# microsoft/Spartan2

Measured on AMD Instinct MI355X. Metric: sha256_spartan prove(): R1CS constraints/sec (prove wall-clock in ms_per_step), higher is better.
Workload: dtype u256 modular integer (8 x u32 Montgomery limbs; T256 scalar/base fields)

## Files before the change

spartan2_amd/csrc/capi_core.hip:

```cpp
#include <atomic>
#include <chrono>
#include <cstdlib>
#include <cstdio>
#include <cstring>

#include "core.hpp"
#include "walk_pool.hpp"
#include "kernels_poly.hpp"
#include "sumcheck_round.hpp"

namespace sp {
static thread_local std::string g_err;
static thread_local sp_wait_hook g_wait_hook = nullptr;
static thread_local void* g_wait_user = nullptr;
void set_error(const std::string& m) { g_err = m; }
static std::atomic<int> g_live_contexts{0};
int live_contexts() { return g_live_contexts.load(std::memory_order_relaxed); }
void relax() {
  if (g_wait_hook) g_wait_hook(g_wait_user);
  else __builtin_ia32_pause();
}
void slow_note(const char* site, long spins) {
  static const bool on = getenv("SPARTAN_SLOWPATH_LOG") != nullptr;
  if (on) fprintf(stderr, "[slow path] %s after %ld polls\n", site, spins);
// ... 501 lines not shown
  if (cap_bytes) *cap_bytes = t->cap * sizeof(fe_t);
  return SP_OK;
}
void sp_table_free(sp_table* t) {
  if (!t) return;
  if (t->d && !t->view) hipFree(t->d);
  delete t;
}

}

static int launch_bind(sp_ctx* c, sp_table** tabs, int nt, const fe_t& r) {
  if (nt > spk::BIND_MAX_TABLES) return fail(SP_ERR_INTERNAL, "launch_bind: too many tables");
  spk::BindArgs a;
  size_t max_eff = 0;
  uint64_t bytes = 0;
  for (int i = 0; i < nt; ++i) {
    sp_table* t = tabs[i];
    if (t->len < 2) return fail(SP_ERR_INVALID_INPUT_LENGTH, "bind_poly_var_top: table must have at least two elements");
    a.z[i] = t->d;
    a.n[i] = t->len / 2;
    a.lo[i] = sp::eff_lo(t);
    a.hi[i] = sp::eff_hi(t);
    size_t eff = sp::eff_pairs(t);
    if (eff > max_eff) max_eff = eff;
    bytes += 48ull * t->len;
  }
  a.r = r;
  a.one_minus_r = fe_sub<S>(fe_one<S>(), r);
  if (max_eff > 0) {
    size_t blocks = (max_eff + 255) / 256;
    if (blocks > 8192) blocks = 8192;
    dim3 grid((unsigned)blocks, (unsigned)nt);
    c->timed("bind", bytes, [&] { hipLaunchKernelGGL(spk::k_bind_top, grid, dim3(256), 0, c->stream, a); });
  }
  for (int i = 0; i < nt; ++i) sp::after_bind(tabs[i]);
  return SP_OK;
}

static unsigned next_seq(sp_ctx* c) { return ++c->result_seq; }
static void reduce_partials_launch(sp_ctx* c, size_t nblocks, int nacc) {
  if (nblocks <= (size_t)spk::HOST_SUM_MAX_BLOCKS) {
    c->pending_slots = (unsigned)nblocks;
    return;
  }
  size_t b2 = (nblocks + 63) / 64;
  if (b2 > (size_t)spk::HOST_SUM_MAX_BLOCKS) b2 = spk::HOST_SUM_MAX_BLOCKS;
  c->pending_slots = (unsigned)b2;
  hipLaunchKernelGGL(spk::k_sum_partials, dim3((unsigned)b2), dim3(64), 0, c->stream, c->d_scratch, nblocks, nacc, c->d_pinned, c->result_seq);
}
static bool fold_stage2_enabled() {
  static const bool on = [] {
    const char* e = getenv("SPARTAN_FOLD_STAGE2");
    return e && e[0] == '1';
  }();
  return on;
}
static spk::LazyOut lazy_out(sp_ctx* c, spk::lazy9_t* lp, size_t nparts, int gl, const fe_t* eq_out, unsigned seq) {
  spk::LazyOut lo(lp);
  const size_t ngroups = nparts >> gl;
  size_t b2 = (ngroups + 63) / 64;
  if (b2 < 1) b2 = 1;
  if (b2 > (size_t)spk::HOST_SUM_MAX_BLOCKS) b2 = spk::HOST_SUM_MAX_BLOCKS;
  lo.eq_out = eq_out;
  lo.mapped = c->d_pinned;
  lo.seq = seq;
  lo.nslots = (unsigned)b2;
  lo.gl = gl;
  static const unsigned fold_slots = [] {
    const char* e = getenv("SPARTAN_FOLD_SLOTS");
    const int v = e ? atoi(e) : spk::HOST_SUM_MAX_BLOCKS;
    return (unsigned)(v < 1 ? 1 : (v > spk::HOST_SUM_MAX_BLOCKS ? spk::HOST_SUM_MAX_BLOCKS : v));
  }();
  size_t fs = fold_slots;
  while (fs > 1 && (fs > ngroups || ngroups % fs)) fs >>= 1;
  const bool even = ngroups > 0 && ((size_t)ngroups << gl) == nparts && ngroups % fs == 0 && (gl == 0 || nparts % 2 == 0);
  if (fold_stage2_enabled() && even && c->d_fold_tickets) {
    lo.tickets = c->d_fold_tickets;
    lo.nslots = (unsigned)fs;
    lo.per_slot = (unsigned)(nparts / fs);
  }
  return lo;
}
static void sum_lazy_launch(sp_ctx* c, const spk::LazyOut& lo, size_t nparts) {
  const int gl = lo.gl;
  const unsigned seq = lo.seq;
  const fe_t* eq_out = lo.eq_out;
  c->pending_slots = lo.nslots;
  if (lo.tickets) return;
  const uint32_t* P = reinterpret_cast<const uint32_t*>(lo.P);
  const dim3 g(lo.nslots), b(64);
  const bool vec_ok = nparts % 8 == 0;
  if (vec_ok && gl == 0) hipLaunchKernelGGL((spk::k_sum_partials_lazy<0>), g, b, 0, c->stream, P, nparts, gl, eq_out, c->d_pinned, seq);
  else if (vec_ok && gl == 1) hipLaunchKernelGGL((spk::k_sum_partials_lazy<1>), g, b, 0, c->stream, P, nparts, gl, eq_out, c->d_pinned, seq);
  else if (vec_ok && gl == 2) hipLaunchKernelGGL((spk::k_sum_partials_lazy<2>), g, b, 0, c->stream, P, nparts, gl, eq_out, c->d_pinned, seq);
  else if (vec_ok && gl == 3) hipLaunchKernelGGL((spk::k_sum_partials_lazy<3>), g, b, 0, c->stream, P, nparts, gl, eq_out, c->d_pinned, seq);
  else hipLaunchKernelGGL((spk::k_sum_partials_lazy<-1>), g, b, 0, c->stream, P, nparts, gl, eq_out, c->d_pinned, seq);
}
static int wait_slot(sp_ctx* c, const fe_t* slot, unsigned want, int nvals, fe_t* v, bool resident, long* spins) {
  volatile const unsigned* fl = reinterpret_cast<volatile const unsigned*>(slot + 3);
  while (*fl != want) {
    if (++*spins > 400000) {
      sp::slow_note("wait_slot", *spins);
      if (resident) {
        const auto t0 = std::chrono::steady_clock::now();
        while (*fl != want) {
          if (std::chrono::steady_clock::now() - t0 > std::chrono::seconds(12)) return fail(SP_ERR_INTERNAL, "sum-check tail kernel did not deliver a round result");
          sp::relax();
        }
        break;
      }
      SP_HIP(sp::stream_sync(c->stream));
      if (*fl != want) return fail(SP_ERR_INTERNAL, "evaluation kernel did not deliver its block sums");
    }
    sp::relax();
  }
  for (long tries = 0;; ++tries) {
    std::atomic_thread_fence(std::memory_order_acquire);
    spk::slot_chk chk = {want, want * spk::SLOT_CHK_K};
    for (int k = 0; k < nvals; ++k) {
      for (int i = 0; i < 8; ++i) v[k].v[i] = reinterpret_cast<volatile const uint32_t*>(slot + k)[i];
      spk::slot_chk_add(chk, v[k], k);
    }
    if (fl[0] == want && fl[1] == chk.a && fl[2] == chk.b && fl[3] == want) return SP_OK;
    if (tries > 4000000) return fail(SP_ERR_INTERNAL, "evaluation kernel delivered an inconsistent result slot");
    sp::relax();
  }
}
int sp::wait_result_slot(sp_ctx* c, const fe_t* slot, unsigned want, int nvals, fe_t* v, long* spins) { return wait_slot(c, slot, want, nvals, v, false, spins); }
static int wait_wide(sp_ctx* c, unsigned want, int nvals, fe_t* v) {
  long spins = 0;
  for (int s0 = 0; s0 < nvals; s0 += 3) {
    int rc = wait_slot(c, c->h_pinned + spk::SLOT_BASE_ELEM + 4 * (s0 / 3), want, nvals - s0 < 3 ? nvals - s0 : 3, v + s0, true, &spins);
    if (rc) return rc;
  }
  return SP_OK;
}
static unsigned host_parts(size_t items, size_t min_per_part) {
  const size_t w = (size_t)sp::WalkPool::get().walkers() + 1;
  size_t p = items / min_per_part;
  if (p > w) p = w;
  if (p > (size_t)sp::WalkPool::MAX_PARTS) p = sp::WalkPool::MAX_PARTS;
  return p ? (unsigned)p : 1u;
}
static int wait_hand_over(sp_ctx* c, unsigned want, int nvals, fe_t* v) {
  long spins = 0;
  const fe_t* area = c->h_pinned + spk::HAND_BASE_ELEM;
  int rc = wait_slot(c, area, want, nvals < 3 ? nvals : 3, v, true, &spins);
  if (rc) return rc;
  for (int s0 = 3; s0 < nvals; s0 += 3) {
    const char* line = reinterpret_cast<const char*>(area + 4 * (s0 / 3));
    __builtin_prefetch(line);
    __builtin_prefetch(line + 64);
  }
  const int nslots = (nvals + 2) / 3;
  if (nslots > 48 && sp::WalkPool::get().walkers() > 0) {
    struct Check {
      sp_ctx* c;
      const fe_t* area;
      unsigned want;
      int nvals, nslots;
      fe_t* v;
      std::atomic<int> rc{SP_OK};
    } ck{c, area, want, nvals, nslots, v};
    auto part = [](void* arg, unsigned p, unsigned np) {
      Check& k = *static_cast<Check*>(arg);
      const int lo = 1 + (int)((long)(k.nslots - 1) * p / np), hi = 1 + (int)((long)(k.nslots - 1) * (p + 1) / np);
      long sp_ = 0;
      for (int sl = lo; sl < hi; ++sl) {
        const int s0 = 3 * sl;
        const int r = wait_slot(k.c, k.area + 4 * sl, k.want, k.nvals - s0 < 3 ? k.nvals - s0 : 3, k.v + s0, true, &sp_);
        if (r) k.rc.store(r, std::memory_order_relaxed);
      }
// ... 782 lines not shown
      }
      return 1;
    }
    if (round + 1 >= rounds) {
      if (ahead) return 0;
      sp_table* tabs[2] = {A, B};
      have_sums = false;
      int rc2 = launch_bind(c, tabs, 2, rv);
      return rc2 ? rc2 : 1;
    }
    const bool gated = ahead && !launch_ahead_ok(c, A->len);
    if (gated && !gate_ok(c)) return 0;
    if (!stopped && tail_enabled() && A->len <= TAIL_MAX_LEN && table_dense(A) && table_dense(B) && lease.take(tail_blocks(A->len / 2))) {
      spk::TailArgs ta;
      ta.A = A->d;
      ta.B = B->d;
      ta.C = nullptr;
      ta.len = A->len;
      ta.r0 = rv;
      ta.eq_pl = ta.eq_pr = nullptr;
      ta.ell = ta.first_half = ta.rnd0 = 0;
      ta.mail = c->d_mail;
      ta.mirror = c->d_mail_mirror;
      ta.r0_from_mail = ahead ? 1 : 0;
      ta.mapped = c->d_pinned;
      ta.seq0 = next_seq(c);
      ta.hand_n = tail_hand_n(false);
      tail_nb0 = tail_blocks(A->len / 2);
      hipLaunchKernelGGL((spk::k_sumcheck_tail<false>), dim3(tail_nb0), dim3(spk::TAIL_THREADS), 0, c->stream, ta);
      if (!c->tail_ev) (void)hipEventCreateWithFlags(&c->tail_ev, hipEventDisableTiming);
      if (c->tail_ev && hipEventRecord(c->tail_ev, c->stream) == hipSuccess) c->tail_ev_pending = true;
      in_tail = true;
      have_sums = true;
      sp::after_bind(A);
      sp::after_bind(B);
      c->pending_slots = tail_blocks(A->len);
      return 1;
    }
    const bool dense = table_dense(A) && table_dense(B);
    const bool sparse_stream = !dense && A->len / 4 >= STREAM_MIN_Q && sp::eff_lo(A) == A->len / 2 && sp::eff_lo(B) == B->len / 2 && sp::eff_hi(A) <= A->len / 4 && sp::eff_hi(B) <= B->len / 4;
    if (gated && !dense && !sparse_stream) return 0;
    const spk::MailRef mref = gated ? gate_launch(c, answers) : mail_ref(c, ahead, answers);
    if (dense) {
      const size_t q = A->len / 4;
      size_t blocks = (q + chunk - 1) / chunk;
      if (q >= STREAM_MIN_Q) {
        const unsigned seq = next_seq(c);
        const spk::LazyOut lp = lazy_out(c, reinterpret_cast<spk::lazy9_t*>(c->d_scratch), q / 256, 2, nullptr, seq);
        c->timed("bind_stream_quad", 48ull * A->len * 2, [&] {
          hipLaunchKernelGGL(spk::k_bind_eval_quad_stream, dim3((unsigned)(q / 256)), dim3(256), 0, c->stream, A->d, B->d, q, rv, lp, mref);
        });
        sum_lazy_launch(c, lp, q / 256);
      } else {
        c->timed("bind", 48ull * A->len * 2, [&] {
          hipLaunchKernelGGL(spk::k_bind_eval_quad, dim3((unsigned)blocks), dim3(256), 0, c->stream, A->d, B->d, q, rv, c->d_scratch, c->d_pinned, next_seq(c), mref);
        });
        reduce_partials_launch(c, blocks, 2);
      }
      sp::after_bind(A);
      sp::after_bind(B);
      have_sums = true;
      return 1;
    }
    if (sparse_stream) {
      const size_t q = A->len / 4;
      const unsigned seq = next_seq(c);
      const spk::LazyOut lp = lazy_out(c, reinterpret_cast<spk::lazy9_t*>(c->d_scratch), q / 256, 2, nullptr, seq);
      c->timed("bind_stream_quad_sparse", 64ull * (A->len / 2) * 2, [&] {
        hipLaunchKernelGGL(spk::k_bind_eval_quad_stream_sparse, dim3((unsigned)(q / 256)), dim3(256), 0, c->stream, A->d, B->d, q, rv, sp::eff_hi(A), sp::eff_hi(B), lp,
                           mref);
      });
      sum_lazy_launch(c, lp, q / 256);
      sp::after_bind(A);
      sp::after_bind(B);
      have_sums = true;
      return 1;
    }
    if (ahead) return 0;
    sp_table* tabs[2] = {A, B};
    have_sums = false;
    int rc2 = launch_bind(c, tabs, 2, rv);
    return rc2 ? rc2 : 1;
  };
  for (size_t round = 0; round < rounds; ++round) {
    const size_t half = A->len / 2, len_now = A->len;
    const double tr0 = round_trace() ? now_us() : 0;
    fe_t sums[2] = {fe_zero(), fe_zero()};
    bool waiting = have_sums;
    if (!have_sums && !host_mode) {
      size_t len = sp::eff_pairs(A);
      if (sp::eff_pairs(B) < len) len = sp::eff_pairs(B);
      if (half < len) len = half;
      if (len >= STREAM_MIN_Q && len % 1024 == 0) {
        const unsigned seq = next_seq(c);
        const size_t hi_max = sp::eff_hi(A) > sp::eff_hi(B) ? sp::eff_hi(A) : sp::eff_hi(B);
        const bool lowhi = hi_max <= len / 2;
        const size_t blocks = len / (256 * (size_t)4);
        const spk::LazyOut lp = lazy_out(c, reinterpret_cast<spk::lazy9_t*>(c->d_scratch), blocks, 2, nullptr, seq);
        c->timed("eval_quad", 64ull * len + 32ull * ((sp::eff_hi(A) < len ? sp::eff_hi(A) : len) + (sp::eff_hi(B) < len ? sp::eff_hi(B) : len)), [&] {
          if (lowhi)
            hipLaunchKernelGGL((spk::k_eval_quad_stream_lowhi<4>), dim3((unsigned)blocks), dim3(256), 0, c->stream, A->d, B->d, half, sp::eff_hi(A), sp::eff_hi(B), lp);
          else
            hipLaunchKernelGGL((spk::k_eval_quad_stream<4>), dim3((unsigned)blocks), dim3(256), 0, c->stream, A->d, B->d, half, sp::eff_hi(A), sp::eff_hi(B), lp);
        });
        sum_lazy_launch(c, lp, blocks);
        waiting = true;
      } else if (len > 0) {
        size_t blocks = (len + chunk - 1) / chunk;
        c->timed("eval_quad", 64ull * len + 32ull * ((sp::eff_hi(A) < len ? sp::eff_hi(A) : len) + (sp::eff_hi(B) < len ? sp::eff_hi(B) : len)),
                 [&] { hipLaunchKernelGGL(spk::k_eval_quad, dim3((unsigned)blocks), dim3(256), 0, c->stream, A->d, B->d, half, len, sp::eff_hi(A), sp::eff_hi(B), c->d_scratch, c->d_pinned, next_seq(c)); });
        reduce_partials_launch(c, blocks, 2);
        waiting = true;
      }
    }
    const unsigned wait_seq = c->result_seq, wait_slots = c->pending_slots;
    const bool wait_resident = in_tail;
    if (wait_resident && !host_mode && spk::tail_hand_over(len_now, tail_hand_n(false))) {
      hA.resize(2 * len_now);
      if ((rc = wait_hand_over(c, wait_seq, (int)(2 * len_now), hA.data()))) return rc;
      hB = hA.data() + len_now;
      host_mode = true;
      hand_seq = wait_seq;
    }
    if (host_mode) {
      host_quad_eval(hA.data(), hB, half, sums);
      waiting = false;
    }
    if (!host_mode && wait_resident && spk::tail_double(false, len_now, tail_hand_n(false))) {
      fe_t S8[8];
      if ((rc = wait_wide(c, wait_seq, spk::TAIL_DOUBLE_SUMS_QUAD, S8))) return rc;
      if (reduce) {
        int hrc = reduce(reduce_user, reinterpret_cast<uint64_t*>(S8), 8);
        if (hrc) return fail(hrc, "prove_quad: the reduce hook failed");
      }
      fe_t rr[2];
      for (int half2 = 0; half2 < 2; ++half2) {
        fe_t e0, tinf;
        if (half2 == 0) {
          e0 = fe_add<S>(S8[0], S8[1]);
          tinf = fe_add<S>(S8[2], S8[3]);
        } else {
          const fe_t r = rr[0];
          e0 = fe_add<S>(S8[0], fe_mul<S>(r, fe_add<S>(fe_sub<S>(fe_sub<S>(S8[4], S8[0]), S8[2]), fe_mul<S>(r, S8[2]))));
          tinf = fe_add<S>(S8[5], fe_mul<S>(r, fe_add<S>(fe_sub<S>(fe_sub<S>(S8[7], S8[5]), S8[6]), fe_mul<S>(r, S8[6]))));
        }
        UniPoly poly;
        poly.n = 3;
        poly.c[0] = e0;
        poly.c[1] = fe_sub<S>(fe_sub<S>(claim, fe_dbl<S>(e0)), tinf);
        poly.c[2] = tinf;
        absorb_poly(tr->t, poly);
        if (!tr->t.squeeze<S>(lbl_c, 1, &rr[half2])) return fail(SP_ERR_INTERNAL_TRANSCRIPT, "transcript round counter overflow");
        tail_post_challenge(c, rr[half2], wait_seq + half2);
        store_fe(out_r + 4 * (round + half2), rr[half2]);
        store_fe(out_cpolys + 8 * (round + half2), poly.c[0]);
        store_fe(out_cpolys + 8 * (round + half2) + 4, poly.c[2]);
        claim = poly_eval(poly, rr[half2]);
      }
      for (int k = 0; k < 2; ++k) {
        sp::after_bind(A);
        sp::after_bind(B);
        next_seq(c);
      }
      have_sums = round + 2 < rounds;
      c->pending_slots = have_sums ? 1u : 0u;
      last_answered = wait_seq + 1;
      guard.armed = round + 2 < rounds;
      if (observe)
        for (int k = 0; k < 2; ++k) {
          uint64_t rw[4];
          store_fe(rw, rr[k]);
          observe(observe_user, round + k, rw);
        }
      if (round_trace()) fprintf(stderr, "quad rounds %2zu+%2zu len %8zu tail 2 wait+host %7.1f us\n", round, round + 1, len_now, now_us() - tr0);
      ++round;
      continue;
    }
    int issued = 0;
    if (!host_mode && waiting && (in_tail || (c->mail_dev && !reduce))) {
      issued = issue(round, nullptr, wait_seq);
      if (issued < 0) return issued;
      guard.armed = issued != 0;
    }
    if (waiting) {
      const unsigned cur_seq = c->result_seq, cur_slots = c->pending_slots;
      c->result_seq = wait_seq;
      c->pending_slots = wait_slots;
      rc = reduce_partials_wait(c, 2, sums, wait_resident || issued != 0);
      if (issued) {
        c->result_seq = cur_seq;
        c->pending_slots = cur_slots;
      }
      if (rc) return rc;
    }
    if (reduce) {
      int hrc = reduce(reduce_user, reinterpret_cast<uint64_t*>(sums), 2);
      if (hrc) return fail(hrc, "prove_quad: the reduce hook failed");
    }
    const double tr1 = round_trace() ? now_us() : 0;
    fe_t e0 = sums[0], tinf = sums[1];
    UniPoly poly;
    poly.n = 3;
    poly.c[0] = e0;
    poly.c[1] = fe_sub<S>(fe_sub<S>(claim, fe_dbl<S>(e0)), tinf);
    poly.c[2] = tinf;
    absorb_poly(tr->t, poly);
    fe_t r_i;
    if (!tr->t.squeeze<S>(lbl_c, 1, &r_i)) return fail(SP_ERR_INTERNAL_TRANSCRIPT, "transcript round counter overflow");
    last_answered = wait_seq;
    if (host_mode) {
      host_bind_tables(hA.data(), (size_t)(hB - hA.data()), 2, len_now, r_i);
      sp::after_bind(A);
      sp::after_bind(B);
      have_sums = false;
    } else if (issued) {
      tail_post_challenge(c, r_i, wait_seq);
    } else {
      issued = issue(round, &r_i, wait_seq);
      if (issued < 0) return issued;
      if (wait_resident) tail_post_challenge(c, r_i, wait_seq);
    }
    store_fe(out_r + 4 * round, r_i);
    store_fe(out_cpolys + 8 * round, poly.c[0]);
    store_fe(out_cpolys + 8 * round + 4, poly.c[2]);
    claim = poly_eval(poly, r_i);
    guard.armed = in_tail && (host_mode || round + 1 < rounds);
    if (observe) {
      uint64_t rw[4];
      store_fe(rw, r_i);
      observe(observe_user, round, rw);
    }
    if (round_trace()) fprintf(stderr, "quad round %2zu len %8zu tail %d wait %7.1f us host %6.1f us\n", round, len_now, (int)wait_resident, tr1 - tr0, now_us() - tr1);
  }
  if (stopped) {
    store_fe(claim_io, claim);
    return tail_check(c);
  }
  if (host_mode) {
    store_fe(out_final, hA[0]);
    store_fe(out_final + 4, hB[0]);
    tail_post_challenge(c, hA[0], hand_seq);
    tail_post_challenge(c, hB[0], hand_seq + 1);
    c->result_seq = hand_seq + 1;
    guard.armed = false;
  } else if (in_tail) {
    fe_t fin[3];
    long spins = 0;
    if ((rc = wait_slot(c, c->h_pinned + spk::TAIL_FINAL_ELEM, last_answered, 2, fin, true, &spins))) return rc;
    store_fe(out_final, fin[0]);
    store_fe(out_final + 4, fin[1]);
  } else {
    rc = sp_table_read(c, A, 0, 1, out_final);
    if (rc) return rc;
    rc = sp_table_read(c, B, 0, 1, out_final + 4);
    if (rc) return rc;
  }
// ... 1077 lines not shown
```

spartan2_amd/csrc/kernels_poly.hpp:

```cpp
#pragma once
#include "device_utils.hpp"
#include "kernels_shared.hpp"

namespace spk {

constexpr int RESULT_FLAG_ELEM = 7;
__device__ __forceinline__ void publish_result(fe_t* result, unsigned seq) {
  __threadfence_system();
  __hip_atomic_store(reinterpret_cast<unsigned*>(result + RESULT_FLAG_ELEM), seq, __ATOMIC_RELEASE, __HIP_MEMORY_SCOPE_SYSTEM);
}

template <int NACC>
__device__ __forceinline__ void emit_partials_wide(const fe_t (&acc)[NACC], fe_t* __restrict__ mapped, unsigned seq);
template <int NACC>
__device__ __forceinline__ void emit_partials(const fe_t (&acc)[NACC], fe_t* __restrict__ partials, fe_t* __restrict__ mapped, unsigned seq) {
  if (gridDim.x <= HOST_SUM_MAX_BLOCKS) {
    fe_t* slot = mapped + SLOT_BASE_ELEM + 4 * blockIdx.x;
    slot_chk chk = {0u, 0u};
#pragma unroll
    for (int k = 0; k < NACC; ++k) {
      slot_store_elem(slot + k, acc[k]);
      slot_chk_add(chk, acc[k], k);
    }
    slot_store_tag(slot, seq, chk);
// ... 488 lines not shown
  bool nz = false;
#pragma unroll
  for (int k = 0; k < PPT; ++k) nz |= !fe_is_zero(p0[k]);
  lazy9_t l0 = lazy_from(fe_zero()), l1 = lazy_from(fe_zero());
#pragma unroll
  for (int k = 0; k < PPT; ++k) l1 = lazy_add(l1, lazy_from(fe_mul<S>(w[k], p1[k])));
  l1 = lazy_wave_sum(l1);
  if (__any(nz)) {
#pragma unroll
    for (int k = 0; k < PPT; ++k) l0 = lazy_add(l0, lazy_from(fe_mul<S>(w[k], p0[k])));
    l0 = lazy_wave_sum(l0);
  }
  stream_block_partials(l0, l1, partials);
}
__global__ void __launch_bounds__(256) k_bind_eval_quad_stream(fe_t* __restrict__ A, fe_t* __restrict__ B, size_t q, fe_t r_arg, LazyOut partials,
                                                               MailRef mref) {
  const size_t id = (size_t)blockIdx.x * blockDim.x + threadIdx.x;
  const fe_t la0 = A[id], la1 = A[id + q], la2 = A[id + 2 * q], la3 = A[id + 3 * q];
  const fe_t lb0 = B[id], lb1 = B[id + q], lb2 = B[id + 2 * q], lb3 = B[id + 3 * q];
  const fe_t r = challenge_or(mref, r_arg);
  const fe_t a0 = bind1(la0, la2, r), a1 = bind1(la1, la3, r);
  const fe_t b0 = bind1(lb0, lb2, r), b1 = bind1(lb1, lb3, r);
  A[id] = a0;
  A[id + q] = a1;
  B[id] = b0;
  B[id + q] = b1;
  stream_block_partials(lazy_wave_sum(lazy_from(fe_mul<S>(a0, b0))), lazy_wave_sum(lazy_from(fe_mul<S>(fe_sub<S>(a1, a0), fe_sub<S>(b1, b0)))), partials);
}
__global__ void __launch_bounds__(256) k_bind_eval_quad_stream_sparse(fe_t* __restrict__ A, fe_t* __restrict__ B, size_t q, fe_t r_arg, size_t hiA, size_t hiB,
                                                                      LazyOut partials, MailRef mref) {
  const size_t id = (size_t)blockIdx.x * blockDim.x + threadIdx.x;
  const fe_t la0 = A[id], la1 = A[id + q], lb0 = B[id], lb1 = B[id + q];
  const fe_t r = challenge_or(mref, r_arg);
  const fe_t one_minus_r = fe_sub<S>(fe_one<S>(), r);
  const fe_t a0 = id < hiA ? bind1(la0, A[id + 2 * q], r) : fe_mul<S>(la0, one_minus_r);
  const fe_t b0 = id < hiB ? bind1(lb0, B[id + 2 * q], r) : fe_mul<S>(lb0, one_minus_r);
  const fe_t a1 = fe_mul<S>(la1, one_minus_r), b1 = fe_mul<S>(lb1, one_minus_r);
  A[id] = a0;
  A[id + q] = a1;
  B[id] = b0;
  B[id + q] = b1;
  stream_block_partials(lazy_wave_sum(lazy_from(fe_mul<S>(a0, b0))), lazy_wave_sum(lazy_from(fe_mul<S>(fe_sub<S>(a1, a0), fe_sub<S>(b1, b0)))), partials);
}
template <int PPT>
__global__ void __launch_bounds__(256) k_eval_quad_stream(const fe_t* __restrict__ A, const fe_t* __restrict__ B, size_t half, size_t hiA, size_t hiB,
                                                          LazyOut partials) {
  const size_t stride = (size_t)gridDim.x * blockDim.x;
  size_t id = (size_t)blockIdx.x * blockDim.x + threadIdx.x;
  lazy9_t l0 = lazy_from(fe_zero()), l1 = lazy_from(fe_zero());
#pragma unroll
  for (int k = 0; k < PPT; ++k, id += stride) {
    const fe_t a0 = A[id], b0 = B[id];
    const fe_t a1 = id < hiA ? A[id + half] : fe_zero(), b1 = id < hiB ? B[id + half] : fe_zero();
    l0 = lazy_add(l0, lazy_from(fe_mul<S>(a0, b0)));
    l1 = lazy_add(l1, lazy_from(fe_mul<S>(fe_sub<S>(a1, a0), fe_sub<S>(b1, b0))));
  }
  stream_block_partials(lazy_wave_sum(l0), lazy_wave_sum(l1), partials);
}
template <int PPT>
__global__ void __launch_bounds__(256) k_eval_quad_stream_lowhi(const fe_t* __restrict__ A, const fe_t* __restrict__ B, size_t half, size_t hiA, size_t hiB,
                                                                LazyOut partials) {
  const size_t stride = (size_t)gridDim.x * blockDim.x;
  const size_t id0 = (size_t)blockIdx.x * blockDim.x + threadIdx.x;
  fe_t a0[PPT], b0[PPT];
#pragma unroll
  for (int k = 0; k < PPT; ++k) {
    a0[k] = A[id0 + k * stride];
    b0[k] = B[id0 + k * stride];
  }
  lazy9_t l0 = lazy_from(fe_zero()), l1 = lazy_from(fe_zero());
#pragma unroll
  for (int k = 0; k < PPT; ++k) {
    const size_t id = id0 + k * stride;
    const fe_t p = fe_mul<S>(a0[k], b0[k]);
    l0 = lazy_add(l0, lazy_from(p));
    if (id < hiA || id < hiB) {
      const fe_t a1 = id < hiA ? A[id + half] : fe_zero(), b1 = id < hiB ? B[id + half] : fe_zero();
      l1 = lazy_add(l1, lazy_from(fe_sub<S>(fe_mul<S>(fe_sub<S>(a1, a0[k]), fe_sub<S>(b1, b0[k])), p)));
    }
  }
  l1 = lazy_add(l1, l0);
  stream_block_partials(lazy_wave_sum(l0), lazy_wave_sum(l1), partials);
}
template <int GL>
__global__ void __launch_bounds__(64) k_sum_partials_lazy(const uint32_t* __restrict__ P, size_t nparts, int gl_rt, const fe_t* __restrict__ eq_out,
                                                          fe_t* __restrict__ mapped, unsigned seq) {
  const int gl = GL >= 0 ? GL : gl_rt;
  const size_t ngroups = nparts >> gl, per = (size_t)1 << gl;
  fe_t acc[2] = {fe_zero(), fe_zero()};
  for (size_t g = (size_t)blockIdx.x * 64 + threadIdx.x; g < ngroups; g += (size_t)gridDim.x * 64) {
    unsigned long long col[2][9];
#pragma unroll
    for (int w = 0; w < 9; ++w)
#pragma unroll
      for (int a = 0; a < 2; ++a) {
        const uint32_t* src = P + (size_t)(2 * w + a) * nparts + g * per;
        if constexpr (GL == 0) {
          col[a][w] = src[0];
        } else if constexpr (GL == 1) {
          const uint2 v = *reinterpret_cast<const uint2*>(src);
          col[a][w] = (unsigned long long)v.x + v.y;
        } else if constexpr (GL == 2) {
          const uint4 v = *reinterpret_cast<const uint4*>(src);
          col[a][w] = ((unsigned long long)v.x + v.y) + ((unsigned long long)v.z + v.w);
        } else if constexpr (GL == 3) {
          const uint4 v = *reinterpret_cast<const uint4*>(src), u = *reinterpret_cast<const uint4*>(src + 4);
          col[a][w] = (((unsigned long long)v.x + v.y) + ((unsigned long long)v.z + v.w)) + (((unsigned long long)u.x + u.y) + ((unsigned long long)u.z + u.w));
        } else {
          unsigned long long t = 0;
          for (size_t k = 0; k < per; ++k) t += src[k];
          col[a][w] = t;
        }
      }
    fe_t f[2];
#pragma unroll
    for (int a = 0; a < 2; ++a) {
      lazy9_t l;
      unsigned long long carry = 0;
#pragma unroll
      for (int w = 0; w < 9; ++w) {
        const unsigned long long t = col[a][w] + carry;
        l.v[w] = (uint32_t)t;
        carry = t >> 32;
      }
      f[a] = lazy_reduce(l);
    }
    if (eq_out) {
      const fe_t eo = eq_out[g];
      f[0] = fe_mul<S>(f[0], eo);
      f[1] = fe_mul<S>(f[1], eo);
    }
    acc[0] = fe_add<S>(acc[0], f[0]);
    acc[1] = fe_add<S>(acc[1], f[1]);
  }
  acc[0] = wave_sum(acc[0]);
  acc[1] = wave_sum(acc[1]);
  if (threadIdx.x == 0) emit_partials<2>(acc, nullptr, mapped, seq);
}

__global__ void __launch_bounds__(256) k_eval_quad(const fe_t* __restrict__ A, const fe_t* __restrict__ B, size_t half, size_t len, size_t hiA, size_t hiB,
                                                   fe_t* __restrict__ partials, fe_t* __restrict__ single_out, unsigned seq) {
  __shared__ fe_t smem[2 * 4];
  const size_t chunk = (size_t)blockDim.x * EVAL_PPT;
  const size_t base = (size_t)blockIdx.x * chunk;
  fe_t acc[2] = {fe_zero(), fe_zero()};
#pragma unroll 1
  for (int k = 0; k < EVAL_PPT; ++k) {
    const size_t id = base + (size_t)k * blockDim.x + threadIdx.x;
    if (id < len) {
      const fe_t a0 = A[id], b0 = B[id];
      const fe_t a1 = id < hiA ? A[id + half] : fe_zero(), b1 = id < hiB ? B[id + half] : fe_zero();
      acc[0] = fe_add<S>(acc[0], fe_mul<S>(a0, b0));
      acc[1] = fe_add<S>(acc[1], fe_mul<S>(fe_sub<S>(a1, a0), fe_sub<S>(b1, b0)));
    }
  }
  block_sum<2>(acc, smem);
  if (threadIdx.x == 0) {
    emit_partials<2>(acc, partials, single_out, seq);
  }
}

template <bool FALLBACK>
__global__ void __launch_bounds__(256) k_eval_cubic_outer_pow(const fe_t* __restrict__ pleft, size_t left, const fe_t* __restrict__ pright, size_t right,
                                                              const fe_t* __restrict__ A, const fe_t* __restrict__ B, const fe_t* __restrict__ C, size_t len,
                                                              fe_t* __restrict__ partials, fe_t* __restrict__ single_out, unsigned seq) {
  __shared__ fe_t smem[3 * 4];
  fe_t acc[3] = {fe_zero(), fe_zero(), fe_zero()};
  const size_t low = (size_t)blockIdx.x * blockDim.x + threadIdx.x;
  if (low < len) {
    fe_t tl, th;
    if (FALLBACK) {
      tl = pleft[low];
      th = pleft[low + len];
    } else {
      const size_t i = low % left, j = low / left;
      const fe_t pl = pleft[i];
      tl = fe_mul<S>(pl, pright[j]);
      th = fe_mul<S>(pl, pright[j + right]);
    }
    const fe_t al = A[low], ah = A[low + len], bl = B[low], bh = B[low + len], cl = C[low], ch = C[low + len];
    acc[0] = fe_mul<S>(tl, fe_sub<S>(fe_mul<S>(al, bl), cl));
    fe_t tb = fe_sub<S>(fe_dbl<S>(th), tl), ab = fe_sub<S>(fe_dbl<S>(ah), al), bb = fe_sub<S>(fe_dbl<S>(bh), bl), cb = fe_sub<S>(fe_dbl<S>(ch), cl);
    acc[1] = fe_mul<S>(tb, fe_sub<S>(fe_mul<S>(ab, bb), cb));
    tb = fe_sub<S>(fe_add<S>(tb, th), tl);
    ab = fe_sub<S>(fe_add<S>(ab, ah), al);
    bb = fe_sub<S>(fe_add<S>(bb, bh), bl);
    cb = fe_sub<S>(fe_add<S>(cb, ch), cl);
    acc[2] = fe_mul<S>(tb, fe_sub<S>(fe_mul<S>(ab, bb), cb));
  }
  block_sum<3>(acc, smem);
  if (threadIdx.x == 0) {
    emit_partials<3>(acc, partials, single_out, seq);
  }
}

struct CubicPairArgs {
  const fe_t *A[2], *B[2], *C[2];
};
template <bool FALLBACK>
__global__ void __launch_bounds__(256) k_eval_cubic_outer_pow_pair(const fe_t* __restrict__ pleft, size_t left, const fe_t* __restrict__ pright, size_t right,
                                                                   CubicPairArgs t, size_t len, unsigned nb, unsigned pp, fe_t* __restrict__ mapped, unsigned seq) {
  __shared__ fe_t smem[3 * 4];
  const unsigned inst = blockIdx.x / nb, bx = blockIdx.x % nb;
  const fe_t* __restrict__ A = t.A[inst];
  const fe_t* __restrict__ B = t.B[inst];
  const fe_t* __restrict__ C = t.C[inst];
  fe_t acc[3] = {fe_zero(), fe_zero(), fe_zero()};
  for (unsigned k = 0; k < pp; ++k) {
    const size_t low = ((size_t)bx * pp + k) * blockDim.x + threadIdx.x;
    if (low >= len) break;
    fe_t tl, th;
    if (FALLBACK) {
      tl = pleft[low];
      th = pleft[low + len];
    } else {
      const size_t i = low % left, j = low / left;
      const fe_t pl = pleft[i];
      tl = fe_mul<S>(pl, pright[j]);
      th = fe_mul<S>(pl, pright[j + right]);
    }
// ... 526 lines not shown
```

Baseline: 997.7 million.

## Fuse first two quad sum-check rounds into one eval pass and double-bind kernel

For the first round of the quadratic sum-check, when the tables have a suitable sparse shape, a new kernel computes the six sums needed for two rounds in a single pass over the data, reduced by a 6-sum variant of the lazy partial reducer. The host then derives both challenges, and a second new kernel binds both variables at once while producing the next round's sums. This removes one full eval/bind pass over the large tables and one host round trip. In exchange it adds special-case code paths, tighter shape conditions, and a refactor of the two-round host logic into a shared lambda.

```diff
diff --git a/spartan2_amd/csrc/capi_core.hip b/spartan2_amd/csrc/capi_core.hip
--- a/spartan2_amd/csrc/capi_core.hip
+++ b/spartan2_amd/csrc/capi_core.hip
@@ -607,13 +607,18 @@
   }
   return lo;
 }
-static void sum_lazy_launch(sp_ctx* c, const spk::LazyOut& lo, size_t nparts) {
+static void sum_lazy_launch(sp_ctx* c, const spk::LazyOut& lo, size_t nparts, int nsums = 2) {
   const int gl = lo.gl;
   const unsigned seq = lo.seq;
   const fe_t* eq_out = lo.eq_out;
+  const uint32_t* P = reinterpret_cast<const uint32_t*>(lo.P);
+  if (nsums == 6) {
+    c->pending_slots = 3 * lo.nslots;
+    hipLaunchKernelGGL((spk::k_sum_partials_lazy<2, 6>), dim3(lo.nslots, 3), dim3(64), 0, c->stream, P, nparts, gl, eq_out, c->d_pinned, seq);
+    return;
+  }
   c->pending_slots = lo.nslots;
   if (lo.tickets) return;
-  const uint32_t* P = reinterpret_cast<const uint32_t*>(lo.P);
   const dim3 g(lo.nslots), b(64);
   const bool vec_ok = nparts % 8 == 0;
   if (vec_ok && gl == 0) hipLaunchKernelGGL((spk::k_sum_partials_lazy<0>), g, b, 0, c->stream, P, nparts, gl, eq_out, c->d_pinned, seq);
@@ -1562,9 +1567,83 @@
     int rc2 = launch_bind(c, tabs, 2, rv);
     return rc2 ? rc2 : 1;
   };
+  auto two_rounds = [&](size_t round, const fe_t* S8, auto&& post, auto&& then) -> int {
+    fe_t rr[2];
+    for (int half2 = 0; half2 < 2; ++half2) {
+      fe_t e0, tinf;
+      if (half2 == 0) {
+        e0 = fe_add<S>(S8[0], S8[1]);
+        tinf = fe_add<S>(S8[2], S8[3]);
+      } else {
+        const fe_t r = rr[0];
+        e0 = fe_add<S>(S8[0], fe_mul<S>(r, fe_add<S>(fe_sub<S>(fe_sub<S>(S8[4], S8[0]), S8[2]), fe_mul<S>(r, S8[2]))));
+        tinf = fe_add<S>(S8[5], fe_mul<S>(r, fe_add<S>(fe_sub<S>(fe_sub<S>(S8[7], S8[5]), S8[6]), fe_mul<S>(r, S8[6]))));
+      }
+      UniPoly poly;
+      poly.n = 3;
+      poly.c[0] = e0;
+      poly.c[1] = fe_sub<S>(fe_sub<S>(claim, fe_dbl<S>(e0)), tinf);
+      poly.c[2] = tinf;
+      absorb_poly(tr->t, poly);
+      if (!tr->t.squeeze<S>(lbl_c, 1, &rr[half2])) return fail(SP_ERR_INTERNAL_TRANSCRIPT, "transcript round counter overflow");
+      post(half2, rr[half2]);
+      store_fe(out_r + 4 * (round + half2), rr[half2]);
+      store_fe(out_cpolys + 8 * (round + half2), poly.c[0]);
+      store_fe(out_cpolys + 8 * (round + half2) + 4, poly.c[2]);
+      claim = poly_eval(poly, rr[half2]);
+    }
+    then(rr);
+    if (observe)
+      for (int k = 0; k < 2; ++k) {
+        uint64_t rw[4];
+        store_fe(rw, rr[k]);
+        observe(observe_user, round + k, rw);
+      }
+    return SP_OK;
+  };
+  const size_t q0 = A->len / 4;
+  const bool two_round_start = !stopped && !reduce && rounds >= 3 && q0 >= STREAM_MIN_Q && q0 % 4096 == 0 && sp::eff_lo(A) == A->len / 2 &&
+                               sp::eff_lo(B) == B->len / 2 && sp::eff_hi(A) <= q0 && sp::eff_hi(B) <= q0;
   for (size_t round = 0; round < rounds; ++round) {
     const size_t half = A->len / 2, len_now = A->len;
     const double tr0 = round_trace() ? now_us() : 0;
+    if (round == 0 && two_round_start) {
+      const size_t q = q0, hiA = sp::eff_hi(A), hiB = sp::eff_hi(B);
+      const size_t eblocks = q / (256 * (size_t)spk::TWO_ROUNDS_PPT);
+      spk::LazyOut ep = lazy_out(c, reinterpret_cast<spk::lazy9_t*>(c->d_scratch), eblocks, 2, nullptr, next_seq(c));
+      ep.tickets = nullptr;
+      if (ep.nslots > 16) ep.nslots = 16;
+      c->timed("eval_quad", 128ull * q + 32ull * (hiA + hiB), [&] {
+        hipLaunchKernelGGL(spk::k_eval_quad_stream_two_rounds, dim3((unsigned)eblocks), dim3(256), 0, c->stream, A->d, B->d, q, hiA, hiB, ep);
+      });
+      sum_lazy_launch(c, ep, eblocks, 6);
+      fe_t S6[6];
+      if ((rc = reduce_partials_wait(c, 2, S6, false, 3))) return rc;
+      const fe_t S8[8] = {S6[0], S6[1], S6[2], S6[1], S6[3], S6[4], S6[5], S6[3]};
+      const unsigned seq0 = c->result_seq;
+      rc = two_rounds(
+          round, S8, [](int, const fe_t&) {},
+          [&](const fe_t* rr) {
+            const fe_t one = fe_one<S>(), omr0 = fe_sub<S>(one, rr[0]);
+            const fe_t omr1 = fe_sub<S>(one, rr[1]), c0 = fe_mul<S>(omr0, omr1), c1 = fe_mul<S>(omr0, rr[1]), c2 = fe_mul<S>(rr[0], omr1);
+            next_seq(c);
+            const spk::LazyOut lp = lazy_out(c, reinterpret_cast<spk::lazy9_t*>(c->d_scratch), q / 512, 2, nullptr, next_seq(c));
+            c->timed("bind_stream_quad_sparse", 96ull * q * 2, [&] {
+              hipLaunchKernelGGL(spk::k_bind2_eval_quad_stream_sparse, dim3((unsigned)(q / 512)), dim3(256), 0, c->stream, A->d, B->d, q, c0, c1, c2, hiA, hiB, lp);
+            });
+            sum_lazy_launch(c, lp, q / 512);
+            for (int k = 0; k < 2; ++k) {
+              sp::after_bind(A);
+              sp::after_bind(B);
+            }
+            have_sums = true;
+            last_answered = seq0 + 1;
+          });
+      if (rc) return rc;
+      if (round_trace()) fprintf(stderr, "quad rounds %2zu+%2zu len %8zu tail 0 start wait+host %7.1f us\n", round, round + 1, len_now, now_us() - tr0);
+      ++round;
+      continue;
+    }
     fe_t sums[2] = {fe_zero(), fe_zero()};
     bool waiting = have_sums;
     if (!have_sums && !host_mode) {
@@ -1613,45 +1692,21 @@
         int hrc = reduce(reduce_user, reinterpret_cast<uint64_t*>(S8), 8);
         if (hrc) return fail(hrc, "prove_quad: the reduce hook failed");
       }
-      fe_t rr[2];
-      for (int half2 = 0; half2 < 2; ++half2) {
-        fe_t e0, tinf;
-        if (half2 == 0) {
-          e0 = fe_add<S>(S8[0], S8[1]);
-          tinf = fe_add<S>(S8[2], S8[3]);
-        } else {
-          const fe_t r = rr[0];
-          e0 = fe_add<S>(S8[0], fe_mul<S>(r, fe_add<S>(fe_sub<S>(fe_sub<S>(S8[4], S8[0]), S8[2]), fe_mul<S>(r, S8[2]))));
-          tinf = fe_add<S>(S8[5], fe_mul<S>(r, fe_add<S>(fe_sub<S>(fe_sub<S>(S8[7], S8[5]), S8[6]), fe_mul<S>(r, S8[6]))));
-        }
-        UniPoly poly;
-        poly.n = 3;
-        poly.c[0] = e0;
-        poly.c[1] = fe_sub<S>(fe_sub<S>(claim, fe_dbl<S>(e0)), tinf);
-        poly.c[2] = tinf;
-        absorb_poly(tr->t, poly);
-        if (!tr->t.squeeze<S>(lbl_c, 1, &rr[half2])) return fail(SP_ERR_INTERNAL_TRANSCRIPT, "transcript round counter overflow");
-        tail_post_challenge(c, rr[half2], wait_seq + half2);
-        store_fe(out_r + 4 * (round + half2), rr[half2]);
-        store_fe(out_cpolys + 8 * (round + half2), poly.c[0]);
-        store_fe(out_cpolys + 8 * (round + half2) + 4, poly.c[2]);
-        claim = poly_eval(poly, rr[half2]);
-      }
-      for (int k = 0; k < 2; ++k) {
-        sp::after_bind(A);
-        sp::after_bind(B);
-        next_seq(c);
-      }
-      have_sums = round + 2 < rounds;
-      c->pending_slots = have_sums ? 1u : 0u;
-      last_answered = wait_seq + 1;
-      guard.armed = round + 2 < rounds;
-      if (observe)
-        for (int k = 0; k < 2; ++k) {
-          uint64_t rw[4];
-          store_fe(rw, rr[k]);
-          observe(observe_user, round + k, rw);
-        }
+      rc = two_rounds(
+          round, S8,
+          [&](int k, const fe_t& r) { tail_post_challenge(c, r, wait_seq + k); },
+          [&](const fe_t*) {
+            for (int k = 0; k < 2; ++k) {
+              sp::after_bind(A);
+              sp::after_bind(B);
+              next_seq(c);
+            }
+            have_sums = round + 2 < rounds;
+            c->pending_slots = have_sums ? 1u : 0u;
+            last_answered = wait_seq + 1;
+            guard.armed = round + 2 < rounds;
+          });
+      if (rc) return rc;
       if (round_trace()) fprintf(stderr, "quad rounds %2zu+%2zu len %8zu tail 2 wait+host %7.1f us\n", round, round + 1, len_now, now_us() - tr0);
       ++round;
       continue;
diff --git a/spartan2_amd/csrc/kernels_poly.hpp b/spartan2_amd/csrc/kernels_poly.hpp
--- a/spartan2_amd/csrc/kernels_poly.hpp
+++ b/spartan2_amd/csrc/kernels_poly.hpp
@@ -594,10 +594,89 @@
   l1 = lazy_add(l1, l0);
   stream_block_partials(lazy_wave_sum(l0), lazy_wave_sum(l1), partials);
 }
-template <int GL>
+template <int NS>
+__device__ __forceinline__ void stream_block_partials_n(const lazy9_t (&sm)[4][NS], LazyOut partials) {
+  __syncthreads();
+  if (threadIdx.x < NS) {
+    const lazy9_t t = lazy_add(lazy_add(sm[0][threadIdx.x], sm[1][threadIdx.x]), lazy_add(sm[2][threadIdx.x], sm[3][threadIdx.x]));
+    uint32_t* P = reinterpret_cast<uint32_t*>(partials.P);
+#pragma unroll
+    for (int w = 0; w < 9; ++w) P[(size_t)(NS * w + threadIdx.x) * gridDim.x + blockIdx.x] = t.v[w];
+  }
+}
+constexpr int TWO_ROUNDS_PPT = 2;
+struct TwoRoundLow {
+  lazy9_t d2, l4, d6;
+};
+__device__ __forceinline__ void two_round_low_terms(TwoRoundLow& t, const fe_t* __restrict__ A, const fe_t* __restrict__ B, size_t id, size_t q, size_t hiA, size_t hiB) {
+  if (id < hiA || id < hiB) {
+    const fe_t a0 = A[id], a1 = A[id + q], b0 = B[id], b1 = B[id + q];
+    const fe_t a2 = id < hiA ? A[id + 2 * q] : fe_zero(), b2 = id < hiB ? B[id + 2 * q] : fe_zero();
+    const fe_t U = fe_sub<S>(a1, a0), V = fe_sub<S>(b1, b0);
+    t.d2 = lazy_add(t.d2, lazy_from(fe_sub<S>(fe_mul<S>(fe_sub<S>(a2, a0), fe_sub<S>(b2, b0)), fe_mul<S>(a0, b0))));
+    t.l4 = lazy_add(t.l4, lazy_from(fe_mul<S>(a2, b2)));
+    t.d6 = lazy_add(t.d6, lazy_from(fe_sub<S>(fe_mul<S>(fe_add<S>(U, a2), fe_add<S>(V, b2)), fe_mul<S>(U, V))));
+  }
+}
+__global__ void __launch_bounds__(256) k_eval_quad_stream_two_rounds(const fe_t* __restrict__ A, const fe_t* __restrict__ B, size_t q, size_t hiA, size_t hiB,
+                                                                     LazyOut partials) {
+  const size_t stride = (size_t)gridDim.x * blockDim.x;
+  const size_t id0 = (size_t)blockIdx.x * blockDim.x + threadIdx.x, id1 = id0 + stride;
+  const fe_t a00 = A[id0], a10 = A[id0 + q], b00 = B[id0], b10 = B[id0 + q];
+  const fe_t a01 = A[id1], a11 = A[id1 + q], b01 = B[id1], b11 = B[id1 + q];
+  __shared__ lazy9_t sm[4][6];
+  const int lane = threadIdx.x & 63, wave = threadIdx.x >> 6;
+  const lazy9_t z = lazy_from(fe_zero());
+  lazy9_t l = lazy_wave_sum(lazy_add(lazy_from(fe_mul<S>(a00, b00)), lazy_from(fe_mul<S>(a01, b01))));
+  if (lane == 0) sm[wave][0] = sm[wave][2] = l;
+  l = lazy_wave_sum(lazy_add(lazy_from(fe_mul<S>(a10, b10)), lazy_from(fe_mul<S>(a11, b11))));
+  if (lane == 0) sm[wave][1] = l;
+  l = lazy_wave_sum(lazy_add(lazy_from(fe_mul<S>(fe_sub<S>(a10, a00), fe_sub<S>(b10, b00))), lazy_from(fe_mul<S>(fe_sub<S>(a11, a01), fe_sub<S>(b11, b01)))));
+  if (lane == 0) {
+    sm[wave][4] = sm[wave][5] = l;
+    sm[wave][3] = z;
+  }
+  const size_t hi = hiA > hiB ? hiA : hiB;
+  if (__any(id0 < hi || id1 < hi)) {
+    TwoRoundLow t = {z, z, z};
+    two_round_low_terms(t, A, B, id0, q, hiA, hiB);
+    two_round_low_terms(t, A, B, id1, q, hiA, hiB);
+    t.d2 = lazy_wave_sum(t.d2);
+    t.l4 = lazy_wave_sum(t.l4);
+    t.d6 = lazy_wave_sum(t.d6);
+    if (lane == 0) {
+      sm[wave][2] = lazy_add(sm[wave][2], t.d2);
+      sm[wave][3] = t.l4;
+      sm[wave][5] = lazy_add(sm[wave][5], t.d6);
+    }
+  }
+  stream_block_partials_n<6>(sm, partials);
+}
+__global__ void __launch_bounds__(256) k_bind2_eval_quad_stream_sparse(fe_t* __restrict__ A, fe_t* __restrict__ B, size_t q, fe_t c0, fe_t c1, fe_t c2, size_t hiA,
+                                                                       size_t hiB, LazyOut partials) {
+  const size_t id = (size_t)blockIdx.x * blockDim.x + threadIdx.x, h = q / 2;
+  const fe_t la0 = A[id], la1 = A[id + q], ma0 = A[id + h], ma1 = A[id + h + q];
+  const fe_t lb0 = B[id], lb1 = B[id + q], mb0 = B[id + h], mb1 = B[id + h + q];
+  fe_t x0 = fe_add<S>(fe_mul<S>(c0, la0), fe_mul<S>(c1, la1)), x1 = fe_add<S>(fe_mul<S>(c0, ma0), fe_mul<S>(c1, ma1));
+  fe_t y0 = fe_add<S>(fe_mul<S>(c0, lb0), fe_mul<S>(c1, lb1)), y1 = fe_add<S>(fe_mul<S>(c0, mb0), fe_mul<S>(c1, mb1));
+  if (id < hiA || id < hiB) {
+    if (id < hiA) x0 = fe_add<S>(x0, fe_mul<S>(c2, A[id + 2 * q]));
+    if (id + h < hiA) x1 = fe_add<S>(x1, fe_mul<S>(c2, A[id + h + 2 * q]));
+    if (id < hiB) y0 = fe_add<S>(y0, fe_mul<S>(c2, B[id + 2 * q]));
+    if (id + h < hiB) y1 = fe_add<S>(y1, fe_mul<S>(c2, B[id + h + 2 * q]));
+  }
+  A[id] = x0;
+  A[id + h] = x1;
+  B[id] = y0;
+  B[id + h] = y1;
+  stream_block_partials(lazy_wave_sum(lazy_from(fe_mul<S>(x0, y0))), lazy_wave_sum(lazy_from(fe_mul<S>(fe_sub<S>(x1, x0), fe_sub<S>(y1, y0)))), partials);
+}
+template <int GL, int NS = 2>
 __global__ void __launch_bounds__(64) k_sum_partials_lazy(const uint32_t* __restrict__ P, size_t nparts, int gl_rt, const fe_t* __restrict__ eq_out,
                                                           fe_t* __restrict__ mapped, unsigned seq) {
+  static_assert(NS >= 2 && NS % 2 == 0, "sums are delivered in pairs");
   const int gl = GL >= 0 ? GL : gl_rt;
+  const int a0 = NS == 2 ? 0 : 2 * (int)blockIdx.y;
   const size_t ngroups = nparts >> gl, per = (size_t)1 << gl;
   fe_t acc[2] = {fe_zero(), fe_zero()};
   for (size_t g = (size_t)blockIdx.x * 64 + threadIdx.x; g < ngroups; g += (size_t)gridDim.x * 64) {
@@ -606,7 +685,7 @@
     for (int w = 0; w < 9; ++w)
 #pragma unroll
       for (int a = 0; a < 2; ++a) {
-        const uint32_t* src = P + (size_t)(2 * w + a) * nparts + g * per;
+        const uint32_t* src = P + (size_t)(NS * w + a0 + a) * nparts + g * per;
         if constexpr (GL == 0) {
           col[a][w] = src[0];
         } else if constexpr (GL == 1) {
@@ -647,7 +726,18 @@
   }
   acc[0] = wave_sum(acc[0]);
   acc[1] = wave_sum(acc[1]);
-  if (threadIdx.x == 0) emit_partials<2>(acc, nullptr, mapped, seq);
+  if (NS == 2) {
+    if (threadIdx.x == 0) emit_partials<2>(acc, nullptr, mapped, seq);
+  } else if (threadIdx.x == 0) {
+    fe_t* slot = mapped + SLOT_BASE_ELEM + 4 * (blockIdx.y * gridDim.x + blockIdx.x);
+    slot_chk chk = {0u, 0u};
+#pragma unroll
+    for (int k = 0; k < 2; ++k) {
+      slot_store_elem(slot + k, acc[k]);
+      slot_chk_add(chk, acc[k], k);
+    }
+    slot_store_tag(slot, seq, chk);
+  }
 }
 
 __global__ void __launch_bounds__(256) k_eval_quad(const fe_t* __restrict__ A, const fe_t* __restrict__ B, size_t half, size_t len, size_t hiA, size_t hiB,
```

New measurement: 1.048 billion (median of 6 runs). +5.1%, better.
